# samson6460/tf2_YOLO

Measured on NVIDIA B200. Metric: images/sec YOLOv4-608 loss+grad+decode+NMS, higher is better.
Workload: dtype f32

## Files before the change

tf2_yolo_b200/csrc/common.cuh:

```cuda
#pragma once
#include <cuda_runtime.h>
#include <stdint.h>

#include "../../include/yolo_b200.h"

namespace yb {
const char*& last_error_site();
}
#define YB_STR2(x) #x
#define YB_STR(x) YB_STR2(x)
#define YB_CUDA_TRY(expr)                                          \
    do {                                                           \
        cudaError_t _e = (expr);                                   \
        if (_e != cudaSuccess) {                                   \
            yb::last_error_site() = __FILE__ ":" YB_STR(__LINE__); \
            (void)cudaGetLastError();  \
            return (int)_e;                                        \
        }                                                          \
    } while (0)

namespace yb {

constexpr int kNumSMs = 148;

// ... 36 lines not shown
__device__ __forceinline__ void bulk_g2s(void* smem_dst, const void* gmem_src, uint32_t bytes,
                                         uint64_t* bar) {
    asm volatile(
        "cp.async.bulk.shared::cluster.global.mbarrier::complete_tx::bytes [%0], [%1], %2, [%3];"
        ::"r"(smem_u32(smem_dst)), "l"(gmem_src), "r"(bytes), "r"(smem_u32(bar))
        : "memory");
}
__device__ __forceinline__ void bulk_s2g(void* gmem_dst, const void* smem_src, uint32_t bytes) {
    asm volatile("cp.async.bulk.global.shared::cta.bulk_group [%0], [%1], %2;" ::"l"(gmem_dst),
                 "r"(smem_u32(smem_src)), "r"(bytes)
                 : "memory");
}
__device__ __forceinline__ void bulk_commit() {
    asm volatile("cp.async.bulk.commit_group;" ::: "memory");
}
template <int N>
__device__ __forceinline__ void bulk_wait_read() {
    asm volatile("cp.async.bulk.wait_group.read %0;" ::"n"(N) : "memory");
}
template <int N>
__device__ __forceinline__ void bulk_wait_all() {
    asm volatile("cp.async.bulk.wait_group %0;" ::"n"(N) : "memory");
}
__device__ __forceinline__ void fence_proxy_async() {
    asm volatile("fence.proxy.async.shared::cta;" ::: "memory");
}

__device__ __forceinline__ void bar_sync(int id, int nthreads) {
    asm volatile("bar.sync %0, %1;" ::"r"(id), "r"(nthreads) : "memory");
}

__device__ __forceinline__ double warp_sum(double v) {
#pragma unroll
    for (int o = 16; o > 0; o >>= 1) v += __shfl_xor_sync(0xffffffffu, v, o);
    return v;
}
__device__ __forceinline__ int warp_sum(int v) {
#pragma unroll
    for (int o = 16; o > 0; o >>= 1) v += __shfl_xor_sync(0xffffffffu, v, o);
    return v;
}

__host__ __device__ __forceinline__ size_t align_up(size_t x, size_t a) {
    return (x + a - 1) / a * a;
}

// ... 17 lines not shown
```

tf2_yolo_b200/csrc/decode.cu:

```cuda
#include <cstring>

#include "common.cuh"
#include "decode_internal.cuh"
#include "scan.cuh"

namespace yb {

constexpr int kDecMaxConsumerWarps = 8;
constexpr int kDecStages = 3;

template <typename T, bool kBuckets>
__global__ void __launch_bounds__((kDecMaxConsumerWarps + 1) * 32)
decode_count_kernel(const __grid_constant__ DecodeLaunch L, const __grid_constant__ DecodeSink K) {
    extern __shared__ __align__(128) unsigned char smem[];
    __shared__ uint64_t full[kDecStages], done[kDecStages];
    const int tid = threadIdx.x, warp = tid >> 5, lane = tid & 31;
    const int ncw = (int)(blockDim.x >> 5) - 1;
    if (tid == 0) {
        for (int i = 0; i < kDecStages; ++i) {
            mbar_init(&full[i], 1);
            mbar_init(&done[i], ncw * 32);
        }
        mbar_fence_init();
    }
// ... 40 lines not shown
                lc = lane / L.B[s];
                lb = lane - lc * L.B[s];
                lane_on = lc < cpw;
            }
            const int B = L.B[s], C = L.C, pcf = L.pcf[s];
            const long long cell0 = (long long)(tile - L.tile_base[s]) * L.tile_cells[s];
            const long long n_cells = L.n_img * L.cells[s];
            const int nc = (int)min((long long)L.tile_cells[s], n_cells - cell0);
            const int stage = it % kDecStages;
            const T* sp = reinterpret_cast<const T*>(smem + (size_t)stage * L.stage_bytes);
            mbar_wait(&full[stage], (it / kDecStages) & 1);
            for (int c0 = warp * cpw; c0 < nc; c0 += ncw * cpw) {
                const int cell = c0 + lc;
                const bool valid = lane_on && cell < nc;
                const int box_at = cell * pcf + lb * ((L.version == 1) ? 5 : 5 + C);
                const int prob_at = (L.version == 1) ? cell * pcf + 5 * B : box_at + 5;
                const T c = valid ? sp[box_at + 4] : (T)0;
                const LaneHits h = decode_count_lane<T>(K, valid, sp + prob_at, c, thr, C, B, lc, lb, s, cell0 + cell);
                if (kBuckets) {
                    T x = 0, y = 0, w = 0, hgt = 0;
                    if (h.n > 0) {
                        x = sp[box_at]; y = sp[box_at + 1]; w = sp[box_at + 2]; hgt = sp[box_at + 3];
                    }
                    decode_file_rows<T>(K.buckets, h, sp, prob_at, lb, x, y, w, hgt, c, thr, C, lane);
                }
            }
            mbar_arrive(&done[stage]);
        }
    }
}

constexpr int kEmitGroup = 8;

template <typename T>
__global__ void __launch_bounds__(256)
decode_emit_kernel(const __grid_constant__ DecodeLaunch L, const unsigned int* __restrict__ n_hot,
                   const HotBox* __restrict__ hot_boxes, const long long* __restrict__ offsets,
                   double* __restrict__ rows, long long cap, long long* __restrict__ row_offsets) {
    const long long tid = (long long)blockIdx.x * blockDim.x + threadIdx.x;
    const long long n_threads = (long long)gridDim.x * blockDim.x;
    const long long per_img = L.cell_base[L.n_scales];
    const T thr = (T)L.thr;
    for (long long i = tid; i <= L.n_img; i += n_threads) row_offsets[i] = offsets[i * per_img];
    const long long n = *n_hot;
    const int sub = threadIdx.x & (kEmitGroup - 1);
    const long long n_groups = n_threads / kEmitGroup;
    const long long rounds = (n + n_groups - 1) / n_groups;
// ... 240 lines not shown
```

tf2_yolo_b200/csrc/decode_internal.cuh:

```cuda
#pragma once
#include "common.cuh"

namespace yb {

struct DecodeLaunch {
    const void* preds[YB_MAX_SCALES];
    int gh[YB_MAX_SCALES], gw[YB_MAX_SCALES], B[YB_MAX_SCALES];
    int pcf[YB_MAX_SCALES];
    long long cells[YB_MAX_SCALES];
    long long cell_base[YB_MAX_SCALES + 1];
    long long scale_base[YB_MAX_SCALES + 1];
    int n_scales, C, version;
    long long n_img;
    double thr;
    int tile_cells[YB_MAX_SCALES];
    int tile_base[YB_MAX_SCALES + 1];
    int bulk_ok[YB_MAX_SCALES];
    int stage_bytes;
};

struct __align__(16) HotBox {
    long long out_idx;
    unsigned int mem_idx;
    unsigned int packed;
// ... 20 lines not shown
    return ((cellpos * 32u + (unsigned)box) << 8) | (unsigned)cls;
}

struct DecodeSink {
    unsigned int* counts;
    unsigned int* n_hot;
    HotBox* hot;
    HotBuckets buckets;
    long long per_img;
    long long cell_base[YB_MAX_SCALES];
    long long cells[YB_MAX_SCALES];
    float thr;
};

template <typename T>
__device__ __forceinline__ T mul_rn(T a, T b);
template <>
__device__ __forceinline__ float mul_rn<float>(float a, float b) { return __fmul_rn(a, b); }
template <>
__device__ __forceinline__ double mul_rn<double>(double a, double b) { return __dmul_rn(a, b); }

struct LaneHits {
    int n;
    unsigned img;
    unsigned cellpos;
    unsigned cis;
    unsigned base;
};

template <typename T>
__device__ __forceinline__ LaneHits decode_count_lane(const DecodeSink& K, bool valid, const T* prob, T c, T thr,
                                                      int C, int B, int lc, int lb, int s, long long g) {
    LaneHits h = {0, 0u, 0u, 0u, 0u};
    if (valid) {
#pragma unroll 16
        for (int k = 0; k < C; ++k) h.n += (mul_rn<T>(c, prob[k]) >= thr) ? 1 : 0;
    }
    int tot = 0, before = 0;
    for (int q = 0; q < B; ++q) {
        const int nq = __shfl_sync(0xffffffffu, h.n, lc * B + q);
        tot += nq;
        before += (q < lb) ? nq : 0;
    }
    if (valid) {
        const long long img = g / K.cells[s];
        const long long o = img * K.per_img + K.cell_base[s] + (g - img * K.cells[s]);
        if (lb == 0 && K.counts != nullptr) K.counts[o] = (unsigned)tot;
        if (h.n > 0 && K.hot != nullptr)
            K.hot[atomicAdd(K.n_hot, 1u)] = make_hot(o, (unsigned)g, s, lb, (unsigned)before);
        h.img = (unsigned)img;
        h.cellpos = (unsigned)(o - img * K.per_img);
        h.cis = ((unsigned)s << 28) | (unsigned)(g - img * K.cells[s]);
        if (K.buckets.n != nullptr && h.n > 0) h.base = atomicAdd(&K.buckets.n[h.img], (unsigned)h.n);
    }
    return h;
}

template <typename T>
__device__ __forceinline__ void decode_file_rows(const HotBuckets& K, const LaneHits& h, const T* tile, int prob_at,
                                                 int lb, T x, T y, T w, T hgt, T c, T thr, int C, int lane) {
    unsigned hot = __ballot_sync(0xffffffffu, h.n > 0);
    while (hot) {
        const int src = __ffs(hot) - 1;
        hot &= hot - 1;
        const int hlb = __shfl_sync(0xffffffffu, lb, src);
        const T* hprob = tile + __shfl_sync(0xffffffffu, prob_at, src);
        const T hc = __shfl_sync(0xffffffffu, c, src);
        const T hx = __shfl_sync(0xffffffffu, x, src), hy = __shfl_sync(0xffffffffu, y, src);
        const T hw = __shfl_sync(0xffffffffu, w, src), hh = __shfl_sync(0xffffffffu, hgt, src);
        const unsigned himg = __shfl_sync(0xffffffffu, h.img, src);
        const unsigned hpos = __shfl_sync(0xffffffffu, h.cellpos, src);
        const unsigned hcis = __shfl_sync(0xffffffffu, h.cis, src);
        unsigned u = __shfl_sync(0xffffffffu, h.base, src);
        FusedRow* dst = K.row + (size_t)himg * K.cap;
        for (int k0 = 0; k0 < C; k0 += 32) {
            const int k = k0 + lane;
            const T p = (k < C) ? hprob[k] : (T)0;
            const bool hit = (k < C) && (mul_rn<T>(hc, p) >= thr);
            const unsigned m = __ballot_sync(0xffffffffu, hit);
            const unsigned at = u + __popc(m & ((1u << lane) - 1u));
            if (hit && at < (unsigned)K.cap) {
                FusedRow fr;
                fr.key = fused_key(hpos, hlb, k);
                fr.x = (float)hx; fr.y = (float)hy; fr.w = (float)hw; fr.h = (float)hh;
                fr.c = (float)hc; fr.p = (float)p;
                fr.cell = hcis;
                dst[at] = fr;
            }
            u += __popc(m);
        }
    }
}

struct DecodeWs {
    unsigned int* n_hot;
    unsigned int* counts;
    long long* offsets;
    HotBox* hot;
    void* scan_ws;
    size_t zero_bytes;
    long long total_cells;
};

int decode_fill(const void* const* preds, int64_t n_img, const yb_decode_params* p, DecodeLaunch& L);
DecodeSink decode_sink(const DecodeLaunch& L, unsigned int* counts, unsigned int* n_hot, HotBox* hot,
                       const HotBuckets& buckets);
int decode_count(DecodeLaunch& L, bool is_f64, const DecodeSink& K, cudaStream_t stream);
int decode_setup(const void* const* preds, int64_t n_img, const yb_decode_params* p, void* workspace,
                 size_t workspace_bytes, DecodeLaunch& L, DecodeWs& ws);
// ... 11 lines not shown
```

tf2_yolo_b200/csrc/loss.cu:

```cuda
#include <cstdlib>
#include <cstring>

#include "common.cuh"
#include "decode_internal.cuh"

namespace yb {

constexpr int kLossMaxConsumerWarps = 8;
constexpr int kLossMaxThreads = (kLossMaxConsumerWarps + 1) * 32;
constexpr int kMaxStages = 4;
constexpr int kTerms = 10;
constexpr int kLossTerms = 5;
constexpr float kEpsF = 1e-07f;
constexpr double kEps = 1e-07;
constexpr int kCtrlWords = 4;

constexpr double kBinHi = 1649267441664.0;
constexpr double kBinLo = 1536.0;
__device__ __forceinline__ void bin_add(double& hi, double& lo, double x) {
    const double h = __dsub_rn(__dadd_rn(x, kBinHi), kBinHi);
    const double r = (h == x) ? 0.0 : __dsub_rn(x, h);
    const double l = __dsub_rn(__dadd_rn(r, kBinLo), kBinLo);
    hi = __dadd_rn(hi, h);
    lo = __dadd_rn(lo, l);
}

struct LossScaleDev {
    const float* y_true;
    const float* y_pred;
    float* dpred;
    long long n_cells;
    int tile_cells;
    int n_tiles;
    int tile_base;
    int pcf, tcf;
    int bulk_ok;
    int B, C;
    float gw, gh;
// ... 101 lines not shown
}

__device__ __forceinline__ void focal_term(float e, float g, float& f, float& df) {
    const float l = logf(1.f - e);
    float eg, eg1;
    if (g == 2.f) {
        eg = e * e;
        eg1 = e;
    } else if (g == 1.f) {
        eg = e;
        eg1 = 1.f;
    } else if (g == 0.f) {
        eg = 1.f;
        eg1 = 0.f;
    } else {
        eg1 = powf(e, g - 1.f);
        eg = eg1 * e;
    }
    f = -eg * l;
    df = -g * eg1 * l + eg / (1.f - e);
}


template <int V, bool kLogits>
__device__ __forceinline__ void class_row(float* q, const float* t, float m, int C, int lane, bool write,
                                          double lwc, double& part) {
    for (int k = lane; k < C; k += 32) {
        const double p = kLogits ? 1.0 / (1.0 + exp(-(double)q[k])) : (double)q[k];
        const double tk = (double)t[k];
        const double pc = fmin(fmax(p, kEps), 1.0 - kEps);
        const double band = (p >= kEps && p <= 1.0 - kEps) ? 1.0 : 0.0;
        double l, g;
        if (V == 1 || V == 2) {
            l = tk * log(pc);
            g = -tk / pc;
        } else {
            l = tk * log(pc) + (1.0 - tk) * log(1.0 - pc);
            g = -(tk / pc - (1.0 - tk) / (1.0 - pc));
        }
        part -= (double)m * l;
        if (write) q[k] = (float)(lwc * (double)m * g * band * (kLogits ? p * (1.0 - p) : 1.0));
    }
}

__device__ __forceinline__ int warp_argmax(const float* v, int C, int lane) {
    float best = -INFINITY;
    int arg = 0x7fffffff;
    for (int k = lane; k < C; k += 32) {
        const float x = v[k];
        if (x > best || arg == 0x7fffffff) {
            best = x;
            arg = k;
        }
    }
#pragma unroll
    for (int o = 16; o > 0; o >>= 1) {
        const float ob = __shfl_xor_sync(0xffffffffu, best, o);
        const int oa = __shfl_xor_sync(0xffffffffu, arg, o);
        if (oa != 0x7fffffff && (arg == 0x7fffffff || ob > best || (ob == best && oa < arg))) {
            best = ob;
            arg = oa;
        }
    }
    return arg;
}

__device__ __forceinline__ float sigmoidf_(float z) { return 1.f / (1.f + expf(-z)); }

#ifdef YB_LOSS_PROFILE
__device__ unsigned long long yb_loss_prof[1024 * 6];
__device__ __forceinline__ unsigned long long gtimer() {
    unsigned long long t;
    asm volatile("mov.u64 %0, %globaltimer;" : "=l"(t));
    return t;
}
#define YB_PROF(slot) do { yb_loss_prof[blockIdx.x * 6 + (slot)] = gtimer(); } while (0)
#else
#define YB_PROF(slot) do { } while (0)
#endif

template <int V, bool kMetrics, bool kDecode, bool kLogits = false>
__global__ void __launch_bounds__(kLossMaxThreads)
loss_fwd_bwd_kernel(const __grid_constant__ LossLaunch L) {
    constexpr int kAcc = kMetrics ? kTerms : kLossTerms;
    extern __shared__ __align__(128) unsigned char smem[];
    const int tid = threadIdx.x;
    const int warp = tid >> 5, lane = tid & 31;
    const int n_stages = L.n_stages;
    const int ncw = (int)(blockDim.x >> 5) - 1;

    unsigned char* ring = smem;
    double* s_acc = reinterpret_cast<double*>(smem + (size_t)n_stages * L.stage_bytes);
    const int n_sc = L.n_scales;
    uint64_t* full = reinterpret_cast<uint64_t*>(s_acc + ncw * n_sc * kTerms * 2);
    uint64_t* done = full + kMaxStages;
    __shared__ int s_is_last;
    __shared__ int s_tile[kMaxStages];

    if (tid == 0) {
        for (int i = 0; i < kMaxStages; ++i) {
            mbar_init(&full[i], 1);
            mbar_init(&done[i], ncw * 32);
        }
        mbar_fence_init();
    }
    for (int i = tid; i < ncw * n_sc * kTerms * 2; i += blockDim.x) s_acc[i] = 0.0;
    __syncthreads();
    if (tid == 0) YB_PROF(0);

    const int total_tiles = L.total_tiles;

    if (warp == ncw) {
        int s_ld = 0, s_st = 0;
        int next = ((int)blockIdx.x < total_tiles) ? (int)blockIdx.x : -1;
        int n_loaded = 0;
        bool end_posted = false;
        for (int t = 0;; ++t) {
            const int stage = t % n_stages;
            const int tile = __shfl_sync(0xffffffffu, next, 0);
            if (tile >= 0) {
                while (tile >= L.sc[s_ld].tile_base + L.sc[s_ld].n_tiles) ++s_ld;
                const LossScaleDev& S = L.sc[s_ld];
                const long long cell0 = (long long)(tile - S.tile_base) * S.tile_cells;
                const int nc = (int)min((long long)S.tile_cells, S.n_cells - cell0);
                float* sp = reinterpret_cast<float*>(ring + (size_t)stage * L.stage_bytes);
                float* st = sp + S.tile_cells * S.pcf;
                const float* gp = S.y_pred + cell0 * S.pcf;
                const float* gt = S.y_true + cell0 * S.tcf;
                if (S.bulk_ok && (nc & 3) == 0) {
                    if (lane == 0) {
                        const uint32_t bp = (uint32_t)nc * S.pcf * 4u, bt = (uint32_t)nc * S.tcf * 4u;
                        s_tile[stage] = tile;
                        mbar_arrive_expect_tx(&full[stage], bp + bt);
                        bulk_g2s(sp, gp, bp, &full[stage]);
                        bulk_g2s(st, gt, bt, &full[stage]);
                    }
                } else {
                    for (int i = lane; i < nc * S.pcf; i += 32) sp[i] = __ldg(gp + i);
                    for (int i = lane; i < nc * S.tcf; i += 32) st[i] = __ldg(gt + i);
                    __syncwarp();
                    if (lane == 0) {
                        s_tile[stage] = tile;
                        mbar_arrive(&full[stage]);
                    }
                }
                ++n_loaded;
                if (lane == 0) {
                    const unsigned tk = atomicAdd(&L.ctrl[1], 1u) + gridDim.x;
                    next = (tk < (unsigned)total_tiles) ? (int)tk : -1;
                }
            } else if (!end_posted) {
                if (lane == 0) {
                    s_tile[stage] = -1;
                    mbar_arrive(&full[stage]);
                }
                end_posted = true;
            }
            const int j = t - (n_stages - 1);
            if (j >= 0 && j < n_loaded) {
                const int jstage = j % n_stages;
                mbar_wait(&done[jstage], (j / n_stages) & 1);
                const int jt = s_tile[jstage];
                while (jt >= L.sc[s_st].tile_base + L.sc[s_st].n_tiles) ++s_st;
                const LossScaleDev& S = L.sc[s_st];
                if (S.dpred != nullptr) {
                    const long long cell0 = (long long)(jt - S.tile_base) * S.tile_cells;
                    const int nc = (int)min((long long)S.tile_cells, S.n_cells - cell0);
                    float* sp = reinterpret_cast<float*>(ring + (size_t)jstage * L.stage_bytes);
                    float* gd = S.dpred + cell0 * S.pcf;
                    if (S.bulk_ok && (nc & 3) == 0) {
                        if (lane == 0) {
                            bulk_s2g(gd, sp, (uint32_t)nc * S.pcf * 4u);
                            bulk_commit();
                            bulk_wait_read<0>();
                        }
                    } else {
                        for (int i = lane; i < nc * S.pcf; i += 32) gd[i] = sp[i];
                    }
                    __syncwarp();
                }
            }
            if (end_posted && j >= n_loaded - 1) break;
        }
        if (lane == 0) YB_PROF(2);
        if (lane == 0) bulk_wait_all<0>();
        if (lane == 0) YB_PROF(3);
    } else {
        double hi[kAcc], lo[kAcc];
#pragma unroll
        for (int k = 0; k < kAcc; ++k) hi[k] = lo[k] = 0.0;
        auto add = [&](int k, double v) { bin_add(hi[k], lo[k], v); };
        int cur = -1;
        int cpw = 0, lc = 0, lb = 0;
        bool lane_on = false;
        float aw = 1.f, ah = 1.f;
        auto flush = [&](int s) {
#pragma unroll
            for (int k = 0; k < kAcc; ++k) {
                const double vh = warp_sum(hi[k]), vl = warp_sum(lo[k]);
                if (lane == 0) {
                    double* a = s_acc + ((warp * n_sc + s) * kTerms + k) * 2;
                    a[0] += vh;
                    a[1] += vl;
                }
                hi[k] = lo[k] = 0.0;
            }
        };

        for (int it = 0;; ++it) {
            const int stage = it % n_stages;
            mbar_wait(&full[stage], (it / n_stages) & 1);
            const int tile = s_tile[stage];
            if (tile < 0) break;
            int s = (cur < 0) ? 0 : cur;
            while (tile >= L.sc[s].tile_base + L.sc[s].n_tiles) ++s;
            if (s != cur) {
                if (cur >= 0) flush(cur);
                cur = s;
                const int Bs = L.sc[s].B;
                cpw = 32 / Bs;
                lc = lane / Bs;
                lb = lane - lc * Bs;
                lane_on = lc < cpw;
                aw = L.sc[s].anc[2 * (lane_on ? lb : 0)];
                ah = L.sc[s].anc[2 * (lane_on ? lb : 0) + 1];
            }
            const LossScaleDev& S = L.sc[s];
            const long long cell0 = (long long)(tile - S.tile_base) * S.tile_cells;
            const int nc = (int)min((long long)S.tile_cells, S.n_cells - cell0);
            float* sp = reinterpret_cast<float*>(ring + (size_t)stage * L.stage_bytes);
            const float* st = sp + S.tile_cells * S.pcf;
            const int B = S.B, C = S.C;
            const int bstride = (V == 1) ? 5 : (5 + C);
            const bool write = S.dpred != nullptr;
            const float inv_n = S.inv_n;

            for (int c0 = warp * cpw; c0 < nc; c0 += ncw * cpw) {
                const int cell = c0 + lc;
                const bool valid = lane_on && cell < nc;
                float* pc = sp + (valid ? cell : c0) * S.pcf + lb * bstride;
                const float* tc = st + (valid ? cell : c0) * S.tcf;
                float px = 0.f, py = 0.f, pw = 1.f, ph = 1.f, c = 0.5f;
                float tx = 0.f, ty = 0.f, tw = 0.f, th = 0.f, obj = 0.f;
                if (valid) {
                    px = pc[0]; py = pc[1]; pw = pc[2]; ph = pc[3]; c = pc[4];
                    tx = tc[0]; ty = tc[1]; tw = tc[2]; th = tc[3]; obj = tc[4];
                    if (kLogits) {
                        px = sigmoidf_(px); py = sigmoidf_(py); c = sigmoidf_(c);
                        pw = aw * expf(pw); ph = ah * expf(ph);
                    }
                }
                const float iou = grid_iou_f32(px, py, pw, ph, tx, ty, tw, th, S.gw, S.gh);
                int amax = 0;
                float best = __shfl_sync(0xffffffffu, iou, lc * B);
                for (int q = 1; q < B; ++q) {
                    const float v = __shfl_sync(0xffffffffu, iou, lc * B + q);
                    if (v > best) {
                        best = v;
                        amax = q;
                    }
                }
                const float resp = (lb == amax) ? 1.f : 0.f;
                const int prob_at = cell * S.pcf + ((V == 1) ? 5 * B : lb * bstride + 5);
                LaneHits dec = {0, 0u, 0u, 0u, 0u};
                if (kDecode)
                    dec = decode_count_lane<float>(L.dec, valid, sp + prob_at, c, L.dec.thr, C, B, lc, lb, s,
                                                   cell0 + cell);
                if (kMetrics) {
                    float cmax = __shfl_sync(0xffffffffu, c, lc * B);
                    for (int q = 1; q < B; ++q) cmax = fmaxf(cmax, __shfl_sync(0xffffffffu, c, lc * B + q));
                    if (valid && lb == 0) {
                        add(kAcc - 5, (obj == ((cmax > 0.5f) ? 1.f : 0.f)) ? 1.0 : 0.0);
                        add(kAcc - 4, (double)(best * obj));
                        add(kAcc - 3, (double)obj);
                    }
                    float eq = 0.f;
                    unsigned om = __ballot_sync(0xffffffffu, valid && obj != 0.f && (V != 1 || lb == 0));
                    while (om) {
                        const int src = __ffs(om) - 1;
                        om &= om - 1;
                        const int rc = __shfl_sync(0xffffffffu, cell, src);
                        const int rb = __shfl_sync(0xffffffffu, lb, src);
                        const float* q = (V == 1) ? sp + rc * S.pcf + 5 * B : sp + rc * S.pcf + rb * bstride + 5;
                        const int ap = warp_argmax(q, C, lane);
                        const int at = warp_argmax(st + rc * S.tcf + 5, C, lane);
                        if (lane == src) eq = (ap == at) ? 1.f : 0.f;
                    }
                    if (V == 1) eq = __shfl_sync(0xffffffffu, eq, lc * B);
                    if (valid && (V != 1 || lb == 0)) add(kAcc - 2, (double)(eq * obj));
                    float hit = iou * (eq * obj);
                    float hmax = __shfl_sync(0xffffffffu, hit, lc * B);
                    for (int q = 1; q < B; ++q) hmax = fmaxf(hmax, __shfl_sync(0xffffffffu, hit, lc * B + q));
                    if (valid && lb == 0) add(kAcc - 1, (hmax >= S.recall_thr) ? 1.0 : 0.0);
                }
                float g0 = 0.f, g1 = 0.f, g2 = 0.f, g3 = 0.f, g4 = 0.f;
                float pos = 0.f;
                if (valid) {
                    if (V == 1) {
                        pos = obj * resp;
                        const float neg = 1.f - pos;
                        const float dx = tx - px, dy = ty - py;
                        add(0, (double)(pos * (dx * dx + dy * dy)));
                        g0 = -2.f * S.lw[0] * pos * dx * inv_n;
                        g1 = -2.f * S.lw[0] * pos * dy * inv_n;
                        const float sw = sqrtf(fmaxf(pw, kEpsF)), sh = sqrtf(fmaxf(ph, kEpsF));
                        const float dw = sqrtf(fmaxf(tw, kEpsF)) - sw, dh = sqrtf(fmaxf(th, kEpsF)) - sh;
                        add(1, (double)(pos * (dw * dw + dh * dh)));
                        g2 = (pw >= kEpsF) ? -S.lw[1] * pos * dw / sw * inv_n : 0.f;
                        g3 = (ph >= kEpsF) ? -S.lw[1] * pos * dh / sh * inv_n : 0.f;
                        if (pos != 0.f) {
                            BoxGrad bg;
                            box_fwd_bwd<false>(px, py, pw, ph, tx, ty, tw, th, S.gw, S.gh, bg);
                            const double d = bg.iou - (double)c;
                            add(2, (double)pos * d * d + (double)(S.bw * neg * c * c));
                            const double gi = 2.0 * S.lw[2] * pos * d * S.inv_n_d;
                            g0 += (float)(gi * bg.diou[0]);
                            g1 += (float)(gi * bg.diou[1]);
                            g2 += (float)(gi * bg.diou[2]);
                            g3 += (float)(gi * bg.diou[3]);
                            g4 = (float)(-gi) + 2.f * S.lw[2] * S.bw * neg * c * inv_n;
                        } else {
                            add(2, (double)(S.bw * neg * c * c));
                            g4 = 2.f * S.lw[2] * S.bw * neg * c * inv_n;
                        }
                    } else {
                        pos = obj * resp;
                        if (V == 4 && S.truth_thr < 1.f)
                            pos = pos + ((iou > S.truth_thr) ? 1.f : 0.f) * (1.f - pos);
                        const float neg = (1.f - pos) * ((iou < S.ignore_thr) ? 1.f : 0.f);
                        const float lpw = logf(pw / aw), lph = logf(ph / ah);
                        if (V == 4) {
                            add(3, (double)(lpw * lpw + lph * lph));
                            g2 = 2.f * S.whw * lpw / pw * inv_n;
                            g3 = 2.f * S.whw * lph / ph * inv_n;
                            const float cc = fminf(fmaxf(c, kEpsF), 1.f - kEpsF);
                            const float band = (c >= kEpsF && c <= 1.f - kEpsF) ? 1.f : 0.f;
                            float e_p, e_n, de_p, de_n;
                            if (S.label_smooth > 0.f) {
                                const float u = 1.f - S.label_smooth - cc, w2 = S.label_smooth - cc;
                                e_p = fabsf(u);
                                de_p = (u > 0.f) ? -1.f : ((u < 0.f) ? 1.f : 0.f);
                                e_n = fabsf(w2);
                                de_n = (w2 > 0.f) ? -1.f : ((w2 < 0.f) ? 1.f : 0.f);
                            } else {
                                e_p = 1.f - cc;
                                de_p = -1.f;
                                e_n = cc;
                                de_n = 1.f;
                            }
                            float fn, dfn;
                            focal_term(e_n, S.gamma, fn, dfn);
                            float lcf = S.bw * neg * fn;
                            float gc = S.bw * neg * dfn * de_n;
                            if (pos != 0.f) {
                                float fp, dfp;
                                focal_term(e_p, S.gamma, fp, dfp);
                                lcf += pos * fp;
                                gc += pos * dfp * de_p;
                                BoxGrad bg;
                                box_fwd_bwd<true>(px, py, pw, ph, tx, ty, tw, th, S.gw, S.gh, bg);
                                add(0, (double)pos * (1.0 - bg.ciou));
                                const double gb = -(double)S.lw[0] * pos * S.inv_n_d;
                                g0 += (float)(gb * bg.dciou[0]);
                                g1 += (float)(gb * bg.dciou[1]);
                                g2 += (float)(gb * bg.dciou[2]);
                                g3 += (float)(gb * bg.dciou[3]);
                            }
                            add(1, (double)lcf);
                            g4 = S.lw[1] * gc * band * inv_n;
                        } else {
                            add(4, (double)(lpw * lpw + lph * lph));
                            g2 = 2.f * S.whw * lpw / pw * inv_n;
                            g3 = 2.f * S.whw * lph / ph * inv_n;
                            if (pos != 0.f) {
                                const float sc = S.use_scale ? (2.f - tw * th) : 1.f;
                                const float dx = tx - px, dy = ty - py;
                                add(0, (double)(pos * sc * (dx * dx + dy * dy)));
                                g0 = -2.f * S.lw[0] * pos * sc * dx * inv_n;
                                g1 = -2.f * S.lw[0] * pos * sc * dy * inv_n;
                                const float dlw = logf(fmaxf(tw / aw, kEpsF)) - lpw;
                                const float dlh = logf(fmaxf(th / ah, kEpsF)) - lph;
                                add(1, (double)(pos * sc * (dlw * dlw + dlh * dlh)));
                                g2 += -2.f * S.lw[1] * pos * sc * dlw / pw * inv_n;
                                g3 += -2.f * S.lw[1] * pos * sc * dlh / ph * inv_n;
// ... 4 lines not shown
                                float fn, dfn;
                                focal_term(cc, S.gamma, fn, dfn);
                                float lcf = S.bw * neg * fn, gc = S.bw * neg * dfn;
                                if (pos != 0.f) {
                                    float fp, dfp;
                                    focal_term(1.f - cc, S.gamma, fp, dfp);
                                    lcf += pos * fp;
                                    gc -= pos * dfp;
                                }
                                add(2, (double)lcf);
                                g4 = S.lw[2] * gc * band * inv_n;
                            } else {
                                const float om = 1.f - c;
                                add(2, (double)(pos * om * om + S.bw * neg * c * c));
                                g4 = S.lw[2] * (-2.f * pos * om + 2.f * S.bw * neg * c) * inv_n;
                            }
                        }
                    }
                    if (kLogits) {
                        g0 *= px * (1.f - px); g1 *= py * (1.f - py); g4 *= c * (1.f - c);
                        g2 *= pw; g3 *= ph;
                    }
                }
                if (kDecode && L.dec.buckets.n != nullptr)
                    decode_file_rows<float>(L.dec.buckets, dec, sp, prob_at, lb, px, py, pw, ph, c, L.dec.thr, C, lane);
                if (valid) {
                    if (write) {
                        pc[0] = g0; pc[1] = g1; pc[2] = g2; pc[3] = g3; pc[4] = g4;
                        if (V != 1 && pos == 0.f) {
                            float* q = pc + 5;
                            for (int k = 0; k < C; ++k) q[k] = 0.f;
                        }
                        if (V == 1 && lb == 0 && obj == 0.f) {
                            float* q = sp + cell * S.pcf + 5 * B;
                            for (int k = 0; k < C; ++k) q[k] = 0.f;
                        }
                    }
                }
                const float rowm = (V == 1) ? ((lb == 0) ? obj : 0.f) : pos;
                unsigned pm = __ballot_sync(0xffffffffu, valid && rowm != 0.f);
                while (pm) {
                    const int src = __ffs(pm) - 1;
                    pm &= pm - 1;
                    const int rc = __shfl_sync(0xffffffffu, cell, src);
                    const int rb = __shfl_sync(0xffffffffu, lb, src);
                    const float m = __shfl_sync(0xffffffffu, rowm, src);
                    float* q = (V == 1) ? sp + rc * S.pcf + 5 * B : sp + rc * S.pcf + rb * bstride + 5;
                    const float* t = st + rc * S.tcf + 5;
                    double part = 0.0;
                    class_row<V, kLogits>(q, t, m, C, lane, write, (double)S.lw[(V == 4) ? 2 : 3] * S.inv_n_d, part);
                    add((V == 4) ? 2 : 3, part);
                }
            }
            fence_proxy_async();
            mbar_arrive(&done[stage]);
        }
        if (cur >= 0) flush(cur);
        if (tid == 0) YB_PROF(1);
    }

    __syncthreads();
    const int n_vals = L.n_scales * kAcc * 2;
    for (int i = tid; i < n_vals; i += (int)blockDim.x) {
        const int s = i / (kAcc * 2), r = i - s * (kAcc * 2);
        double v = 0.0;
        for (int w = 0; w < ncw; ++w) v += s_acc[(w * n_sc + s) * kTerms * 2 + r];
        if (v != 0.0) atomicAdd(&L.gacc[i], v);
    }
    __threadfence();
    __syncthreads();
    if (tid == 0) s_is_last = (atomicAdd(&L.ctrl[0], 1u) == gridDim.x - 1);
    __syncthreads();
    if (tid == 0) YB_PROF(4);
    if (!s_is_last) return;
    __threadfence();
    double* s_fin = s_acc;
    for (int i = tid; i < L.n_scales * kAcc; i += (int)blockDim.x) {
        const int s = i / kAcc, k = i - s * kAcc;
        const double vh = __ldcg(&L.gacc[2 * i]), vl = __ldcg(&L.gacc[2 * i + 1]);
        L.gacc[2 * i] = 0.0;
        L.gacc[2 * i + 1] = 0.0;
// ... 37 lines not shown
                                int ps, long long n_boxes, int B, float gw, float gh,
                                float* __restrict__ iou_out, float* __restrict__ ciou_out) {
    const long long i = (long long)blockIdx.x * blockDim.x + threadIdx.x;
    if (i >= n_boxes) return;
    const long long cell = i / B;
    const float* t = bt + cell * ts;
    const float* p = bp + i * ps;
    const float iou = grid_iou_f32(p[0], p[1], p[2], p[3], t[0], t[1], t[2], t[3], gw, gh);
    iou_out[i] = iou;
    if (ciou_out != nullptr) {
        BoxGrad bg;
        box_fwd_bwd<true>(p[0], p[1], p[2], p[3], t[0], t[1], t[2], t[3], gw, gh, bg);
        ciou_out[i] = (float)bg.ciou;
    }
}


struct LossEnv {
    int stages, ctas_per_sm, tile_cells, warps;
    static int get(const char* name, int dflt) {
        const char* v = getenv(name);
        return (v && *v) ? atoi(v) : dflt;
    }
    LossEnv() : stages(get("YB_LOSS_STAGES", 2)), ctas_per_sm(get("YB_LOSS_CTAS_PER_SM", 4)),
                tile_cells(get("YB_LOSS_TILE_CELLS", 0)), warps(get("YB_LOSS_WARPS", 0)) {}
};
static const LossEnv& loss_env() {
    static const LossEnv e;
    return e;
}

static size_t loss_gacc_bytes(int n_scales) {
    return align_up((size_t)n_scales * kTerms * 2 * sizeof(double), 256);
}

static int fill_scale(const yb_loss_scale& in, LossScaleDev& d) {
    const yb_loss_params& p = in.p;
    if (in.y_true == nullptr || in.y_pred == nullptr) return YB_E_NULL;
    if (p.version < 1 || p.version > 4) return YB_E_PARAM;
    if (p.grid_h <= 0 || p.grid_w <= 0 || p.bbox_num <= 0 || p.bbox_num > YB_MAX_BOXES ||
        p.class_num <= 0 || in.n_cells < 0)
        return YB_E_SHAPE;
    if (((uintptr_t)in.y_true | (uintptr_t)in.y_pred | (uintptr_t)in.dpred) & 3) return YB_E_ALIGN;
    d.y_true = in.y_true;
    d.y_pred = in.y_pred;
    d.dpred = in.dpred;
    d.n_cells = in.n_cells;
// ... 12 lines not shown
    d.truth_thr = p.truth_thresh;
    d.label_smooth = p.label_smooth;
    d.gamma = p.focal_gamma;
    d.use_focal = p.use_focal;
    d.use_scale = (p.version == 2) ? 1 : p.use_scale;
    d.inv_n = (float)p.inv_batch;
    d.inv_n_d = p.inv_batch;
    for (int k = 0; k < kLossTerms; ++k) d.term_w[k] = 0.0;
    d.recall_thr = 0.5f;
    if (p.version == 4) {
        d.whw = p.wh_reg_weight;
        d.term_w[0] = p.loss_weight[0];
        d.term_w[1] = p.loss_weight[1];
        d.term_w[2] = p.loss_weight[2];
        d.term_w[3] = p.wh_reg_weight;
    } else {
        d.whw = (p.version == 1) ? 0.f : 0.01f;
        for (int k = 0; k < 4; ++k) d.term_w[k] = p.loss_weight[k];
        d.term_w[4] = (p.version == 1) ? 0.0 : 0.01;
    }
    return YB_OK;
}

template <int V, bool kMetrics, bool kDecode>
static int launch_loss_variant(const LossLaunch& L, int grid, int threads, size_t smem, cudaStream_t stream) {
    static SmemRaised done;
    YB_CUDA_TRY(raise_dynamic_smem_once(loss_fwd_bwd_kernel<V, kMetrics, kDecode>, (int)smem, &done));
    loss_fwd_bwd_kernel<V, kMetrics, kDecode><<<grid, threads, smem, stream>>>(L);
    YB_CUDA_TRY(cudaGetLastError());
    return YB_OK;
}

template <int V, bool kMetrics>
static int launch_loss_logits(const LossLaunch& L, int grid, int threads, size_t smem, cudaStream_t stream) {
    static SmemRaised done;
    YB_CUDA_TRY(raise_dynamic_smem_once(loss_fwd_bwd_kernel<V, kMetrics, false, true>, (int)smem, &done));
    loss_fwd_bwd_kernel<V, kMetrics, false, true><<<grid, threads, smem, stream>>>(L);
    YB_CUDA_TRY(cudaGetLastError());
    return YB_OK;
}

template <int V>
static int launch_loss(const LossLaunch& L, bool d, int grid, int threads, size_t smem, cudaStream_t stream) {
    const bool m = L.metrics_out != nullptr;
    if (L.from_logits) {
        if (V != 3 && V != 4) return YB_E_PARAM;
        if (d) return YB_E_PARAM;
        if (V == 3 || V == 4) {
            constexpr int W = (V == 3 || V == 4) ? V : 4;
            return m ? launch_loss_logits<W, true>(L, grid, threads, smem, stream)
                     : launch_loss_logits<W, false>(L, grid, threads, smem, stream);
        }
    }
    if (m && d) return launch_loss_variant<V, true, true>(L, grid, threads, smem, stream);
    if (m) return launch_loss_variant<V, true, false>(L, grid, threads, smem, stream);
    if (d) return launch_loss_variant<V, false, true>(L, grid, threads, smem, stream);
    return launch_loss_variant<V, false, false>(L, grid, threads, smem, stream);
}

}

using namespace yb;

#ifdef YB_LOSS_PROFILE
extern "C" int yb_debug_loss_profile(unsigned long long* host_out) {
    return (int)cudaMemcpyFromSymbol(host_out, yb::yb_loss_prof, sizeof(unsigned long long) * 1024 * 6);
}
#endif

extern "C" size_t yb_loss_workspace_bytes(int n_scales) {
    if (n_scales < 1) n_scales = 1;
    if (n_scales > YB_MAX_SCALES) n_scales = YB_MAX_SCALES;
    return loss_gacc_bytes(n_scales) + 256;
}

static int loss_impl(const yb_loss_scale* scales, int n_scales, float* loss_out, double* terms_out,
                     double* metrics_out, double recall_iou_threshold, void* workspace,
                     size_t workspace_bytes, yb_stream_t stream_, const DecodeSink* dec = nullptr,
                     bool workspace_is_clean = false) {
    cudaStream_t stream = reinterpret_cast<cudaStream_t>(stream_);
    if (scales == nullptr || loss_out == nullptr || workspace == nullptr) return YB_E_NULL;
    if (n_scales < 1 || n_scales > YB_MAX_SCALES) return YB_E_SHAPE;
    if (workspace_bytes < yb_loss_workspace_bytes(n_scales) || ((uintptr_t)workspace & 255))
        return YB_E_WORKSPACE;

    LossLaunch L;
    memset(&L, 0, sizeof(L));
    L.n_scales = n_scales;
    const int version = scales[0].p.version;
    L.from_logits = scales[0].p.from_logits ? 1 : 0;
    int cell_bytes_max = 0;
    for (int s = 0; s < n_scales; ++s) {
        if (scales[s].p.version != version) return YB_E_PARAM;
        if ((scales[s].p.from_logits ? 1 : 0) != L.from_logits) return YB_E_PARAM;
        int rc = fill_scale(scales[s], L.sc[s]);
        if (rc != YB_OK) return rc;
        cell_bytes_max = max(cell_bytes_max, (L.sc[s].pcf + L.sc[s].tcf) * 4);
    }

    int n_stages = loss_env().stages;
    n_stages = max(2, min(kMaxStages, n_stages));
    int ctas_per_sm = max(1, min(8, loss_env().ctas_per_sm));
    const int tile_env = loss_env().tile_cells;
    const size_t sm_smem = 228 * 1024, static_smem = 192;
    auto acc_bytes = [&](int warps) { return sizeof(double) * warps * n_scales * kTerms * 2; };
    const size_t bar_bytes = 2 * kMaxStages * sizeof(uint64_t);
    int total_tiles = 0, stage_bytes = 0, ncw = kLossMaxConsumerWarps;
    for (int pass = 0; pass < 2; ++pass) {
        int stage_budget = 0;
        for (;;) {
            const size_t per_cta = sm_smem / ctas_per_sm - 1024 - static_smem - acc_bytes(ncw) - bar_bytes;
            stage_budget = (int)(per_cta / n_stages) / 128 * 128;
            if (stage_budget >= 4 * cell_bytes_max) break;
            if (ctas_per_sm > 1) {
                --ctas_per_sm;
            } else if (n_stages > 2) {
                --n_stages;
            } else {
                return YB_E_SHAPE;
            }
        }
        total_tiles = 0;
        stage_bytes = 0;
        int warps = 1;
        for (int s = 0; s < n_scales; ++s) {
            LossScaleDev& d = L.sc[s];
            const int cb = (d.pcf + d.tcf) * 4;
            const int cpw = 32 / d.B;
            int t = stage_budget / cb / 4 * 4;
            t = min(t, kLossMaxConsumerWarps * cpw / 4 * 4);
            if (tile_env > 0) t = min(t, tile_env / 4 * 4);
            t = max(4, t);
            d.tile_cells = t;
            d.n_tiles = (int)((d.n_cells + t - 1) / t);
            d.tile_base = total_tiles;
            total_tiles += d.n_tiles;
            stage_bytes = max(stage_bytes, (int)align_up((size_t)t * cb, 128));
            warps = max(warps, min(kLossMaxConsumerWarps, (t + cpw - 1) / cpw));
        }
        ncw = max(1, min(kLossMaxConsumerWarps, (loss_env().warps > 0 ? loss_env().warps : warps)));
    }
    L.total_tiles = total_tiles;
    L.stage_bytes = stage_bytes;
    L.n_stages = n_stages;
    L.gacc = reinterpret_cast<double*>(workspace);
    L.ctrl = reinterpret_cast<unsigned int*>((char*)workspace + loss_gacc_bytes(n_scales));
    L.loss_out = loss_out;
    L.terms_out = terms_out;
    L.metrics_out = metrics_out;
    for (int s = 0; s < n_scales; ++s) L.sc[s].recall_thr = (float)recall_iou_threshold;
// ... 193 lines not shown
```

Measured before the change: 319,900.

## Stage only y_true box heads in smem and read class rows from global on demand

The loss producer warp now copies only the first five y_true fields per cell into shared memory using per-element cp.async with an mbarrier arrive, instead of bulk-copying the whole target row. Class targets are read directly from global memory (with L2 prefetch for positive cells) only for rows that need them. Because each stage holds less data, tiles can be larger or more CTAs can fit per SM, and the default CTAs per SM rises to 5. The change also sets a register-capped launch bound for non-metric variants and clamps the grid to resident occupancy. Rare accumulations are warp-reduced only when needed, and decode recomputes cell placement rather than carrying it in registers. The risks are many small scattered 4-byte async copies in place of one contiguous bulk copy, and extra global latency for class rows.

Result: slower. 265,500, median of 6 (-17.0%).

```diff
diff --git a/tf2_yolo_b200/csrc/common.cuh b/tf2_yolo_b200/csrc/common.cuh
--- a/tf2_yolo_b200/csrc/common.cuh
+++ b/tf2_yolo_b200/csrc/common.cuh
@@ -82,6 +82,14 @@
 __device__ __forceinline__ void bulk_wait_all() {
     asm volatile("cp.async.bulk.wait_group %0;" ::"n"(N) : "memory");
 }
+__device__ __forceinline__ void cp_async_4(void* smem_dst, const void* gmem_src) {
+    asm volatile("cp.async.ca.shared.global [%0], [%1], 4;" ::"r"(smem_u32(smem_dst)), "l"(gmem_src)
+                 : "memory");
+}
+__device__ __forceinline__ void cp_async_mbar_arrive(uint64_t* bar) {
+    asm volatile("cp.async.mbarrier.arrive.shared::cta.b64 [%0];" ::"r"(smem_u32(bar)) : "memory");
+}
+
 __device__ __forceinline__ void fence_proxy_async() {
     asm volatile("fence.proxy.async.shared::cta;" ::: "memory");
 }
diff --git a/tf2_yolo_b200/csrc/decode.cu b/tf2_yolo_b200/csrc/decode.cu
--- a/tf2_yolo_b200/csrc/decode.cu
+++ b/tf2_yolo_b200/csrc/decode.cu
@@ -86,7 +86,7 @@
                     if (h.n > 0) {
                         x = sp[box_at]; y = sp[box_at + 1]; w = sp[box_at + 2]; hgt = sp[box_at + 3];
                     }
-                    decode_file_rows<T>(K.buckets, h, sp, prob_at, lb, x, y, w, hgt, c, thr, C, lane);
+                    decode_file_rows<T>(K, h, s, cell0 + cell, sp, prob_at, lb, x, y, w, hgt, c, thr, C, lane);
                 }
             }
             mbar_arrive(&done[stage]);
diff --git a/tf2_yolo_b200/csrc/decode_internal.cuh b/tf2_yolo_b200/csrc/decode_internal.cuh
--- a/tf2_yolo_b200/csrc/decode_internal.cuh
+++ b/tf2_yolo_b200/csrc/decode_internal.cuh
@@ -66,16 +66,27 @@
 
 struct LaneHits {
     int n;
-    unsigned img;
-    unsigned cellpos;
-    unsigned cis;
     unsigned base;
 };
+
+struct CellPlace {
+    long long img, o;
+    unsigned cellpos, cis;
+};
+__device__ __forceinline__ CellPlace cell_place(const DecodeSink& K, int s, long long g) {
+    CellPlace p;
+    p.img = g / K.cells[s];
+    const long long in_scale = g - p.img * K.cells[s];
+    p.o = p.img * K.per_img + K.cell_base[s] + in_scale;
+    p.cellpos = (unsigned)(K.cell_base[s] + in_scale);
+    p.cis = ((unsigned)s << 28) | (unsigned)in_scale;
+    return p;
+}
 
 template <typename T>
 __device__ __forceinline__ LaneHits decode_count_lane(const DecodeSink& K, bool valid, const T* prob, T c, T thr,
                                                       int C, int B, int lc, int lb, int s, long long g) {
-    LaneHits h = {0, 0u, 0u, 0u, 0u};
+    LaneHits h = {0, 0u};
     if (valid) {
 #pragma unroll 16
         for (int k = 0; k < C; ++k) h.n += (mul_rn<T>(c, prob[k]) >= thr) ? 1 : 0;
@@ -87,22 +98,20 @@
         before += (q < lb) ? nq : 0;
     }
     if (valid) {
-        const long long img = g / K.cells[s];
-        const long long o = img * K.per_img + K.cell_base[s] + (g - img * K.cells[s]);
-        if (lb == 0 && K.counts != nullptr) K.counts[o] = (unsigned)tot;
+        const CellPlace p = cell_place(K, s, g);
+        if (lb == 0 && K.counts != nullptr) K.counts[p.o] = (unsigned)tot;
         if (h.n > 0 && K.hot != nullptr)
-            K.hot[atomicAdd(K.n_hot, 1u)] = make_hot(o, (unsigned)g, s, lb, (unsigned)before);
-        h.img = (unsigned)img;
-        h.cellpos = (unsigned)(o - img * K.per_img);
-        h.cis = ((unsigned)s << 28) | (unsigned)(g - img * K.cells[s]);
-        if (K.buckets.n != nullptr && h.n > 0) h.base = atomicAdd(&K.buckets.n[h.img], (unsigned)h.n);
+            K.hot[atomicAdd(K.n_hot, 1u)] = make_hot(p.o, (unsigned)g, s, lb, (unsigned)before);
+        if (K.buckets.n != nullptr && h.n > 0) h.base = atomicAdd(&K.buckets.n[p.img], (unsigned)h.n);
     }
     return h;
 }
 
 template <typename T>
-__device__ __forceinline__ void decode_file_rows(const HotBuckets& K, const LaneHits& h, const T* tile, int prob_at,
-                                                 int lb, T x, T y, T w, T hgt, T c, T thr, int C, int lane) {
+__device__ __forceinline__ void decode_file_rows(const DecodeSink& D, const LaneHits& h, int s, long long g,
+                                                 const T* tile, int prob_at, int lb, T x, T y, T w, T hgt, T c,
+                                                 T thr, int C, int lane) {
+    const HotBuckets& K = D.buckets;
     unsigned hot = __ballot_sync(0xffffffffu, h.n > 0);
     while (hot) {
         const int src = __ffs(hot) - 1;
@@ -112,11 +121,9 @@
         const T hc = __shfl_sync(0xffffffffu, c, src);
         const T hx = __shfl_sync(0xffffffffu, x, src), hy = __shfl_sync(0xffffffffu, y, src);
         const T hw = __shfl_sync(0xffffffffu, w, src), hh = __shfl_sync(0xffffffffu, hgt, src);
-        const unsigned himg = __shfl_sync(0xffffffffu, h.img, src);
-        const unsigned hpos = __shfl_sync(0xffffffffu, h.cellpos, src);
-        const unsigned hcis = __shfl_sync(0xffffffffu, h.cis, src);
+        const CellPlace hp = cell_place(D, s, __shfl_sync(0xffffffffu, g, src));
         unsigned u = __shfl_sync(0xffffffffu, h.base, src);
-        FusedRow* dst = K.row + (size_t)himg * K.cap;
+        FusedRow* dst = K.row + (size_t)hp.img * K.cap;
         for (int k0 = 0; k0 < C; k0 += 32) {
             const int k = k0 + lane;
             const T p = (k < C) ? hprob[k] : (T)0;
@@ -125,10 +132,10 @@
             const unsigned at = u + __popc(m & ((1u << lane) - 1u));
             if (hit && at < (unsigned)K.cap) {
                 FusedRow fr;
-                fr.key = fused_key(hpos, hlb, k);
+                fr.key = fused_key(hp.cellpos, hlb, k);
                 fr.x = (float)hx; fr.y = (float)hy; fr.w = (float)hw; fr.h = (float)hh;
                 fr.c = (float)hc; fr.p = (float)p;
-                fr.cell = hcis;
+                fr.cell = hp.cis;
                 dst[at] = fr;
             }
             u += __popc(m);
diff --git a/tf2_yolo_b200/csrc/loss.cu b/tf2_yolo_b200/csrc/loss.cu
--- a/tf2_yolo_b200/csrc/loss.cu
+++ b/tf2_yolo_b200/csrc/loss.cu
@@ -1,3 +1,4 @@
+#include <atomic>
 #include <cstdlib>
 #include <cstring>
 
@@ -8,12 +9,14 @@
 
 constexpr int kLossMaxConsumerWarps = 8;
 constexpr int kLossMaxThreads = (kLossMaxConsumerWarps + 1) * 32;
+constexpr int kLossRegCapThreads = 512;
 constexpr int kMaxStages = 4;
 constexpr int kTerms = 10;
 constexpr int kLossTerms = 5;
 constexpr float kEpsF = 1e-07f;
 constexpr double kEps = 1e-07;
 constexpr int kCtrlWords = 4;
+constexpr int kHead = 5;
 
 constexpr double kBinHi = 1649267441664.0;
 constexpr double kBinLo = 1536.0;
@@ -161,12 +164,17 @@
 }
 
 
+__device__ __forceinline__ void prefetch_class_row(const float* t, int C) {
+    for (int k = 0; k < C; k += 32) asm volatile("prefetch.global.L2 [%0];" ::"l"(t + k));
+    asm volatile("prefetch.global.L2 [%0];" ::"l"(t + C - 1));
+}
+
 template <int V, bool kLogits>
 __device__ __forceinline__ void class_row(float* q, const float* t, float m, int C, int lane, bool write,
                                           double lwc, double& part) {
     for (int k = lane; k < C; k += 32) {
         const double p = kLogits ? 1.0 / (1.0 + exp(-(double)q[k])) : (double)q[k];
-        const double tk = (double)t[k];
+        const double tk = (double)__ldg(t + k);
         const double pc = fmin(fmax(p, kEps), 1.0 - kEps);
         const double band = (p >= kEps && p <= 1.0 - kEps) ? 1.0 : 0.0;
         double l, g;
@@ -182,11 +190,12 @@
     }
 }
 
+template <bool kGlobal>
 __device__ __forceinline__ int warp_argmax(const float* v, int C, int lane) {
     float best = -INFINITY;
     int arg = 0x7fffffff;
     for (int k = lane; k < C; k += 32) {
-        const float x = v[k];
+        const float x = kGlobal ? __ldg(v + k) : v[k];
         if (x > best || arg == 0x7fffffff) {
             best = x;
             arg = k;
@@ -207,19 +216,27 @@
 __device__ __forceinline__ float sigmoidf_(float z) { return 1.f / (1.f + expf(-z)); }
 
 #ifdef YB_LOSS_PROFILE
-__device__ unsigned long long yb_loss_prof[1024 * 6];
+constexpr int kProfSlots = 10;
+__device__ unsigned long long yb_loss_prof[1024 * kProfSlots];
 __device__ __forceinline__ unsigned long long gtimer() {
     unsigned long long t;
     asm volatile("mov.u64 %0, %globaltimer;" : "=l"(t));
     return t;
 }
-#define YB_PROF(slot) do { yb_loss_prof[blockIdx.x * 6 + (slot)] = gtimer(); } while (0)
+#define YB_PROF(slot) do { yb_loss_prof[blockIdx.x * kProfSlots + (slot)] = gtimer(); } while (0)
+#define YB_PROF_CLEAR_TOTALS() \
+    do { for (int _k = 6; _k < kProfSlots; ++_k) yb_loss_prof[blockIdx.x * kProfSlots + _k] = 0ull; } while (0)
+#define YB_PROF_TIMED(acc, stmt) do { const long long _c0 = clock64(); stmt; acc += clock64() - _c0; } while (0)
+#define YB_PROF_ADD(slot, v) atomicAdd(&yb_loss_prof[blockIdx.x * kProfSlots + (slot)], (unsigned long long)(v))
 #else
 #define YB_PROF(slot) do { } while (0)
+#define YB_PROF_CLEAR_TOTALS() do { } while (0)
+#define YB_PROF_TIMED(acc, stmt) do { stmt; } while (0)
+#define YB_PROF_ADD(slot, v) do { } while (0)
 #endif
 
 template <int V, bool kMetrics, bool kDecode, bool kLogits = false>
-__global__ void __launch_bounds__(kLossMaxThreads)
+__global__ void __launch_bounds__(kMetrics ? kLossMaxThreads : kLossRegCapThreads)
 loss_fwd_bwd_kernel(const __grid_constant__ LossLaunch L) {
     constexpr int kAcc = kMetrics ? kTerms : kLossTerms;
     extern __shared__ __align__(128) unsigned char smem[];
@@ -242,12 +259,17 @@
             mbar_init(&done[i], ncw * 32);
         }
         mbar_fence_init();
+        YB_PROF_CLEAR_TOTALS();
     }
     for (int i = tid; i < ncw * n_sc * kTerms * 2; i += blockDim.x) s_acc[i] = 0.0;
     __syncthreads();
     if (tid == 0) YB_PROF(0);
 
     const int total_tiles = L.total_tiles;
+#ifdef YB_LOSS_PROFILE
+    long long prof_wait = 0;
+    const long long prof_t0 = clock64();
+#endif
 
     if (warp == ncw) {
         int s_ld = 0, s_st = 0;
@@ -267,16 +289,24 @@
                 const float* gp = S.y_pred + cell0 * S.pcf;
                 const float* gt = S.y_true + cell0 * S.tcf;
                 if (S.bulk_ok && (nc & 3) == 0) {
+                    for (int i = lane; i < nc * kHead; i += 32) {
+                        const int c = i / kHead;
+                        cp_async_4(st + i, gt + (long long)c * S.tcf + (i - c * kHead));
+                    }
+                    cp_async_mbar_arrive(&full[stage]);
+                    __syncwarp();
                     if (lane == 0) {
-                        const uint32_t bp = (uint32_t)nc * S.pcf * 4u, bt = (uint32_t)nc * S.tcf * 4u;
+                        const uint32_t bp = (uint32_t)nc * S.pcf * 4u;
                         s_tile[stage] = tile;
-                        mbar_arrive_expect_tx(&full[stage], bp + bt);
+                        mbar_arrive_expect_tx(&full[stage], bp);
                         bulk_g2s(sp, gp, bp, &full[stage]);
-                        bulk_g2s(st, gt, bt, &full[stage]);
                     }
                 } else {
                     for (int i = lane; i < nc * S.pcf; i += 32) sp[i] = __ldg(gp + i);
-                    for (int i = lane; i < nc * S.tcf; i += 32) st[i] = __ldg(gt + i);
+                    for (int i = lane; i < nc * kHead; i += 32) {
+                        const int c = i / kHead;
+                        st[i] = __ldg(gt + (long long)c * S.tcf + (i - c * kHead));
+                    }
                     __syncwarp();
                     if (lane == 0) {
                         s_tile[stage] = tile;
@@ -298,7 +328,7 @@
             const int j = t - (n_stages - 1);
             if (j >= 0 && j < n_loaded) {
                 const int jstage = j % n_stages;
-                mbar_wait(&done[jstage], (j / n_stages) & 1);
+                YB_PROF_TIMED(prof_wait, mbar_wait(&done[jstage], (j / n_stages) & 1));
                 const int jt = s_tile[jstage];
                 while (jt >= L.sc[s_st].tile_base + L.sc[s_st].n_tiles) ++s_st;
                 const LossScaleDev& S = L.sc[s_st];
@@ -321,7 +351,11 @@
             }
             if (end_posted && j >= n_loaded - 1) break;
         }
-        if (lane == 0) YB_PROF(2);
+        if (lane == 0) {
+            YB_PROF(2);
+            YB_PROF_ADD(8, prof_wait);
+            YB_PROF_ADD(9, clock64() - prof_t0);
+        }
         if (lane == 0) bulk_wait_all<0>();
         if (lane == 0) YB_PROF(3);
     } else {
@@ -345,10 +379,21 @@
                 hi[k] = lo[k] = 0.0;
             }
         };
+        auto add_rare = [&](int k, double v) {
+            double h = 0.0, l = 0.0;
+            bin_add(h, l, v);
+            h = warp_sum(h);
+            l = warp_sum(l);
+            if (lane == 0) {
+                double* a = s_acc + ((warp * n_sc + cur) * kTerms + k) * 2;
+                a[0] += h;
+                a[1] += l;
+            }
+        };
 
         for (int it = 0;; ++it) {
             const int stage = it % n_stages;
-            mbar_wait(&full[stage], (it / n_stages) & 1);
+            YB_PROF_TIMED(prof_wait, mbar_wait(&full[stage], (it / n_stages) & 1));
             const int tile = s_tile[stage];
             if (tile < 0) break;
             int s = (cur < 0) ? 0 : cur;
@@ -378,7 +423,7 @@
                 const int cell = c0 + lc;
                 const bool valid = lane_on && cell < nc;
                 float* pc = sp + (valid ? cell : c0) * S.pcf + lb * bstride;
-                const float* tc = st + (valid ? cell : c0) * S.tcf;
+                const float* tc = st + (valid ? cell : c0) * kHead;
                 float px = 0.f, py = 0.f, pw = 1.f, ph = 1.f, c = 0.5f;
                 float tx = 0.f, ty = 0.f, tw = 0.f, th = 0.f, obj = 0.f;
                 if (valid) {
@@ -401,7 +446,7 @@
                 }
                 const float resp = (lb == amax) ? 1.f : 0.f;
                 const int prob_at = cell * S.pcf + ((V == 1) ? 5 * B : lb * bstride + 5);
-                LaneHits dec = {0, 0u, 0u, 0u, 0u};
+                LaneHits dec = {0, 0u};
                 if (kDecode)
                     dec = decode_count_lane<float>(L.dec, valid, sp + prob_at, c, L.dec.thr, C, B, lc, lb, s,
                                                    cell0 + cell);
@@ -421,8 +466,8 @@
                         const int rc = __shfl_sync(0xffffffffu, cell, src);
                         const int rb = __shfl_sync(0xffffffffu, lb, src);
                         const float* q = (V == 1) ? sp + rc * S.pcf + 5 * B : sp + rc * S.pcf + rb * bstride + 5;
-                        const int ap = warp_argmax(q, C, lane);
-                        const int at = warp_argmax(st + rc * S.tcf + 5, C, lane);
+                        const int ap = warp_argmax<false>(q, C, lane);
+                        const int at = warp_argmax<true>(S.y_true + (cell0 + rc) * S.tcf + kHead, C, lane);
                         if (lane == src) eq = (ap == at) ? 1.f : 0.f;
                     }
                     if (V == 1) eq = __shfl_sync(0xffffffffu, eq, lc * B);
@@ -434,9 +479,11 @@
                 }
                 float g0 = 0.f, g1 = 0.f, g2 = 0.f, g3 = 0.f, g4 = 0.f;
                 float pos = 0.f;
+                double box_term = 0.0;
                 if (valid) {
                     if (V == 1) {
                         pos = obj * resp;
+                        if (lb == 0 && obj != 0.f) prefetch_class_row(S.y_true + (cell0 + cell) * S.tcf + kHead, C);
                         const float neg = 1.f - pos;
                         const float dx = tx - px, dy = ty - py;
                         add(0, (double)(pos * (dx * dx + dy * dy)));
@@ -466,6 +513,7 @@
                         pos = obj * resp;
                         if (V == 4 && S.truth_thr < 1.f)
                             pos = pos + ((iou > S.truth_thr) ? 1.f : 0.f) * (1.f - pos);
+                        if (pos != 0.f) prefetch_class_row(S.y_true + (cell0 + cell) * S.tcf + kHead, C);
                         const float neg = (1.f - pos) * ((iou < S.ignore_thr) ? 1.f : 0.f);
                         const float lpw = logf(pw / aw), lph = logf(ph / ah);
                         if (V == 4) {
@@ -498,7 +546,7 @@
                                 gc += pos * dfp * de_p;
                                 BoxGrad bg;
                                 box_fwd_bwd<true>(px, py, pw, ph, tx, ty, tw, th, S.gw, S.gh, bg);
-                                add(0, (double)pos * (1.0 - bg.ciou));
+                                box_term = (double)pos * (1.0 - bg.ciou);
                                 const double gb = -(double)S.lw[0] * pos * S.inv_n_d;
                                 g0 += (float)(gb * bg.dciou[0]);
                                 g1 += (float)(gb * bg.dciou[1]);
@@ -549,8 +597,10 @@
                         g2 *= pw; g3 *= ph;
                     }
                 }
+                if (V == 4 && __any_sync(0xffffffffu, valid && pos != 0.f)) add_rare(0, box_term);
                 if (kDecode && L.dec.buckets.n != nullptr)
-                    decode_file_rows<float>(L.dec.buckets, dec, sp, prob_at, lb, px, py, pw, ph, c, L.dec.thr, C, lane);
+                    decode_file_rows<float>(L.dec, dec, s, cell0 + cell, sp, prob_at, lb, px, py, pw, ph, c, L.dec.thr, C,
+                                            lane);
                 if (valid) {
                     if (write) {
                         pc[0] = g0; pc[1] = g1; pc[2] = g2; pc[3] = g3; pc[4] = g4;
@@ -573,10 +623,13 @@
                     const int rb = __shfl_sync(0xffffffffu, lb, src);
                     const float m = __shfl_sync(0xffffffffu, rowm, src);
                     float* q = (V == 1) ? sp + rc * S.pcf + 5 * B : sp + rc * S.pcf + rb * bstride + 5;
-                    const float* t = st + rc * S.tcf + 5;
+                    const float* t = S.y_true + (cell0 + rc) * S.tcf + kHead;
                     double part = 0.0;
                     class_row<V, kLogits>(q, t, m, C, lane, write, (double)S.lw[(V == 4) ? 2 : 3] * S.inv_n_d, part);
-                    add((V == 4) ? 2 : 3, part);
+                    if (V == 4)
+                        add_rare(2, part);
+                    else
+                        add(3, part);
                 }
             }
             fence_proxy_async();
@@ -584,6 +637,10 @@
         }
         if (cur >= 0) flush(cur);
         if (tid == 0) YB_PROF(1);
+        if (lane == 0) {
+            YB_PROF_ADD(6, prof_wait);
+            YB_PROF_ADD(7, clock64() - prof_t0);
+        }
     }
 
     __syncthreads();
@@ -667,7 +724,7 @@
         const char* v = getenv(name);
         return (v && *v) ? atoi(v) : dflt;
     }
-    LossEnv() : stages(get("YB_LOSS_STAGES", 2)), ctas_per_sm(get("YB_LOSS_CTAS_PER_SM", 4)),
+    LossEnv() : stages(get("YB_LOSS_STAGES", 2)), ctas_per_sm(get("YB_LOSS_CTAS_PER_SM", 5)),
                 tile_cells(get("YB_LOSS_TILE_CELLS", 0)), warps(get("YB_LOSS_WARPS", 0)) {}
 };
 static const LossEnv& loss_env() {
@@ -726,10 +783,27 @@
     return YB_OK;
 }
 
+template <typename K>
+static cudaError_t clamp_to_resident(K kernel, int threads, size_t smem, std::atomic<unsigned long long>* cache,
+                                     int& grid) {
+    const unsigned long long key = ((unsigned long long)smem << 16) | (unsigned)threads;
+    unsigned long long c = cache->load(std::memory_order_acquire);
+    int per_sm = (int)(c >> 48);
+    if (per_sm == 0 || (c & 0xffffffffffffull) != key) {
+        cudaError_t e = cudaOccupancyMaxActiveBlocksPerMultiprocessor(&per_sm, kernel, threads, smem);
+        if (e != cudaSuccess) return e;
+        cache->store(((unsigned long long)per_sm << 48) | key, std::memory_order_release);
+    }
+    grid = max(1, min(grid, per_sm * kNumSMs));
+    return cudaSuccess;
+}
+
 template <int V, bool kMetrics, bool kDecode>
 static int launch_loss_variant(const LossLaunch& L, int grid, int threads, size_t smem, cudaStream_t stream) {
     static SmemRaised done;
+    static std::atomic<unsigned long long> resident{0};
     YB_CUDA_TRY(raise_dynamic_smem_once(loss_fwd_bwd_kernel<V, kMetrics, kDecode>, (int)smem, &done));
+    YB_CUDA_TRY(clamp_to_resident(loss_fwd_bwd_kernel<V, kMetrics, kDecode>, threads, smem, &resident, grid));
     loss_fwd_bwd_kernel<V, kMetrics, kDecode><<<grid, threads, smem, stream>>>(L);
     YB_CUDA_TRY(cudaGetLastError());
     return YB_OK;
@@ -738,7 +812,9 @@
 template <int V, bool kMetrics>
 static int launch_loss_logits(const LossLaunch& L, int grid, int threads, size_t smem, cudaStream_t stream) {
     static SmemRaised done;
+    static std::atomic<unsigned long long> resident{0};
     YB_CUDA_TRY(raise_dynamic_smem_once(loss_fwd_bwd_kernel<V, kMetrics, false, true>, (int)smem, &done));
+    YB_CUDA_TRY(clamp_to_resident(loss_fwd_bwd_kernel<V, kMetrics, false, true>, threads, smem, &resident, grid));
     loss_fwd_bwd_kernel<V, kMetrics, false, true><<<grid, threads, smem, stream>>>(L);
     YB_CUDA_TRY(cudaGetLastError());
     return YB_OK;
@@ -768,7 +844,7 @@
 
 #ifdef YB_LOSS_PROFILE
 extern "C" int yb_debug_loss_profile(unsigned long long* host_out) {
-    return (int)cudaMemcpyFromSymbol(host_out, yb::yb_loss_prof, sizeof(unsigned long long) * 1024 * 6);
+    return (int)cudaMemcpyFromSymbol(host_out, yb::yb_loss_prof, sizeof(yb::yb_loss_prof));
 }
 #endif
 
@@ -799,7 +875,7 @@
         if ((scales[s].p.from_logits ? 1 : 0) != L.from_logits) return YB_E_PARAM;
         int rc = fill_scale(scales[s], L.sc[s]);
         if (rc != YB_OK) return rc;
-        cell_bytes_max = max(cell_bytes_max, (L.sc[s].pcf + L.sc[s].tcf) * 4);
+        cell_bytes_max = max(cell_bytes_max, (L.sc[s].pcf + kHead) * 4);
     }
 
     int n_stages = loss_env().stages;
@@ -829,7 +905,7 @@
         int warps = 1;
         for (int s = 0; s < n_scales; ++s) {
             LossScaleDev& d = L.sc[s];
-            const int cb = (d.pcf + d.tcf) * 4;
+            const int cb = (d.pcf + kHead) * 4;
             const int cpw = 32 / d.B;
             int t = stage_budget / cb / 4 * 4;
             t = min(t, kLossMaxConsumerWarps * cpw / 4 * 4);
```
